# EtherealEngine/Universal-Volumetric

Measured on AMD Instinct MI355X. Metric: frames/s encode, 100k-vert mesh + 2048^2 texture, higher is better.
Workload: dtype u8/int32 (f32 only in the quantiser)

## Files before the change

### universal-volumetric_amd/csrc/tex_encode.hip

```cpp
#include "uvol_common.hpp"
#include "tex_device.hpp"
#include <algorithm>

#define TJOB_OR_RETURN TexJob &J = job[blockIdx.z]; if (J.status != 0) return
#define TEX_RETRY_ALPHA (~(size_t)0)

__device__ inline uint32_t t_block_excl_scan(uint32_t v, uint32_t *total) {
  __shared__ uint32_t wsum[UVOL_BLOCK / 64];
  const int lane = threadIdx.x & 63, w = threadIdx.x >> 6;
  uint32_t x = v;
  for (int d = 1; d < 64; d <<= 1) { uint32_t y = __shfl_up(x, d); if (lane >= d) x += y; }
  if (lane == 63) wsum[w] = x;
  __syncthreads();
  uint32_t base = 0, tot = 0;
  for (int i = 0; i < UVOL_BLOCK / 64; i++) { if (i < w) base += wsum[i]; tot += wsum[i]; }
  __syncthreads();
  *total = tot;
  return base + x - v;
}
__global__ void __launch_bounds__(UVOL_BLOCK) k_tscan_a(TexJob *job, uint32_t n) {
  TexJob &J = job[blockIdx.z];
  const uint32_t i = blockIdx.x * UVOL_BLOCK + threadIdx.x;
  uint32_t v = (J.status == 0 && i < n) ? J.flag[i] : 0, tot;
  t_block_excl_scan(v, &tot);
  if (threadIdx.x == 0) J.bsum[blockIdx.x] = tot;
}
__global__ void __launch_bounds__(UVOL_BLOCK) k_tscan_b(TexJob *job, uint32_t nblocks) {
  TexJob &J = job[blockIdx.z];
  __shared__ uint32_t carry;
  if (threadIdx.x == 0) carry = 0;
  __syncthreads();
  for (uint32_t b0 = 0; b0 < nblocks; b0 += UVOL_BLOCK) {
    const uint32_t i = b0 + threadIdx.x;
    uint32_t v = i < nblocks ? J.bsum[i] : 0, tot;
    const uint32_t ex = t_block_excl_scan(v, &tot);
    const uint32_t c = carry;
    if (i < nblocks) J.bsum[i] = c + ex;
    __syncthreads();
    if (threadIdx.x == 0) carry = c + tot;
    __syncthreads();
  }
  if (threadIdx.x == 0) J.bsum[nblocks] = carry;
}

__global__ void __launch_bounds__(UVOL_BLOCK) k_tex_skip(TexJob *job) {
  TJOB_OR_RETURN;
  const uint32_t b = blockIdx.x * UVOL_BLOCK + threadIdx.x;
  if (b >= J.nb) return;
  const uint32_t X = b % J.bx, Y = b / J.bx;
  uint32_t anchor[16], cur[16], amask = 0xff000000u;
  const uint32_t st = 1u << J.ashift;
  for (uint32_t kind = 0; kind < st; kind++) {
    t_load_block(J, kind, X, Y, anchor, &amask);
    J.skip[(size_t)kind * J.nb + b] = 0; J.flag[(size_t)kind * J.nb + b] = 1;
    for (uint32_t l = kind + st; l < J.L; l += st) {
      t_load_block(J, l, X, Y, cur, &amask);
      uint32_t d = 0;
      for (int i = 0; i < 16; i++) {
        const int dr = (int)(cur[i] & 255) - (int)(anchor[i] & 255), dg = (int)((cur[i] >> 8) & 255) - (int)((anchor[i] >> 8) & 255), db = (int)((cur[i] >> 16) & 255) - (int)((anchor[i] >> 16) & 255);
        d += (uint32_t)(dr * dr + dg * dg + db * db);
      }
      const bool sk = d <= J.T_skip;
      J.skip[(size_t)l * J.nb + b] = sk ? 1 : 0; J.flag[(size_t)l * J.nb + b] = sk ? 0 : 1;
      if (!sk) for (int i = 0; i < 16; i++) anchor[i] = cur[i];
    }
  }
  if (!J.ashift && (amask & 0xff000000u) != 0xff000000u) J.status = TEX_E_ALPHA;
}

__global__ void __launch_bounds__(UVOL_BLOCK) k_tex_fit(TexJob *job) {
  TJOB_OR_RETURN;
  const uint32_t it = blockIdx.x * UVOL_BLOCK + threadIdx.x;
  if (it >= J.n_items) return;
  const uint32_t b = J.item[it];
  const uint32_t l = b / J.nb, r = b % J.nb;
  uint32_t px[16]; t_load_block(J, l, r % J.bx, r / J.bx, px);
  int sum[3] = {0, 0, 0};
  for (int i = 0; i < 16; i++) { sum[0] += (int)(px[i] & 255); sum[1] += (int)((px[i] >> 8) & 255); sum[2] += (int)((px[i] >> 16) & 255); }
  int base5[3]; for (int c = 0; c < 3; c++) base5[c] = (((sum[c] + 8) >> 4) * 31 + 127) / 255;
  uint32_t best = 0xffffffffu; int bc0 = 0, bc1 = 0, bc2 = 0, bt = 0;
  for (int t = 0; t < 8; t++) for (int di = 0; di < 3; di++) {
    const int dd = di == 0 ? 0 : (di == 1 ? -1 : 1);
    const int c0 = t_clampi(base5[0] + dd, 0, 31), c1 = t_clampi(base5[1] + dd, 0, 31), c2 = t_clampi(base5[2] + dd, 0, 31);
    const uint32_t e = t_eval_block<false, false>(px, c0, c1, c2, t, nullptr, nullptr);
    if (e < best) { best = e; bt = t; bc0 = c0; bc1 = c1; bc2 = c2; }
  }
  for (int c = 0; c < 3; c++) for (int di = 1; di < 3; di++) {
    const int dd = di == 1 ? -1 : 1;
    int c0 = bc0 + (c == 0 ? dd : 0), c1 = bc1 + (c == 1 ? dd : 0), c2 = bc2 + (c == 2 ? dd : 0);
    const int cc = c == 0 ? c0 : (c == 1 ? c1 : c2);
    if (cc < 0 || cc > 31) continue;
    const uint32_t e = t_eval_block<false, false>(px, c0, c1, c2, bt, nullptr, nullptr);
    if (e < best) { best = e; bc0 = c0; bc1 = c1; bc2 = c2; }
  }
  const uint32_t cell = ((uint32_t)bt << 15) | ((uint32_t)bc0 << 10) | ((uint32_t)bc1 << 5) | (uint32_t)bc2;
  J.cell[b] = cell;
  atomicAdd(&J.hist[cell], 1u);
}

__global__ void __launch_bounds__(UVOL_BLOCK) k_cell_flags(TexJob *job) {
  TJOB_OR_RETURN;
  const uint32_t c = blockIdx.x * UVOL_BLOCK + threadIdx.x;
  if (c < (1u << 18)) J.flag[c] = J.hist[c] ? 1 : 0;
}
__global__ void __launch_bounds__(UVOL_BLOCK) k_cell_compact(TexJob *job) {
  TexJob &J = job[blockIdx.z];
  const uint32_t c = blockIdx.x * UVOL_BLOCK + threadIdx.x;
  const bool live = J.status == 0 && c < (1u << 18);
  uint32_t v = live ? J.flag[c] : 0, tot;
  const uint32_t pos = t_block_excl_scan(v, &tot) + J.bsum[blockIdx.x];
  if (live && v) { J.cid[pos] = c; J.cw[pos] = J.hist[c]; J.cidx[c] = pos; }
  if (blockIdx.x == 0 && threadIdx.x == 0 && J.status == 0) {
    const uint32_t n = J.bsum[(1u << 18) / UVOL_BLOCK];
    J.ncell = n;
    TexVQ &V = J.vq[0]; V.n_items = n; V.K = n < J.Kmax_e ? n : J.Kmax_e; V.nl = 1; V.done = (V.K <= 1) ? 1 : 0;
  }
}

template <int DIM> __device__ __forceinline__ void vq_item(const TexJob &J, uint32_t i, int x[DIM], unsigned long long &w) {
  if (DIM == 4) { t_cell_coords(J.cid[i], x); w = J.cw[i]; }
  else { const uint32_t s = J.bsel[J.item[i]]; for (int k = 0; k < DIM; k++) x[k] = (int)((s >> (2 * k)) & 3); w = 1; }
}
template <int DIM> __device__ __forceinline__ int vq_wd(int d) { return (DIM == 4 && d == 3) ? 2 : 1; }

template <int DIM>
__global__ void __launch_bounds__(UVOL_BLOCK) k_vq_zero(TexJob *job, int force) {
  TJOB_OR_RETURN;
  TexVQ &V = J.vq[DIM == 4 ? 0 : 1];
  if (V.done && !force) return;
  const uint32_t i = blockIdx.x * UVOL_BLOCK + threadIdx.x;
// ... 236 lines not shown
  }
  if (live) V.leaf[i] = bk;
}

__global__ void __launch_bounds__(UVOL_BLOCK) k_unique(TexJob *job, int which) {
  TJOB_OR_RETURN;
  const uint32_t K = J.vq[which].nl;
  const uint32_t *val = which == 0 ? J.ent : J.scb;
  uint32_t *outv = which == 0 ? J.ecb : J.scu, *map = which == 0 ? J.emap : J.smap;
  uint8_t *first = J.vq[which].splittable;
  __shared__ uint32_t s_cnt;
  if (threadIdx.x == 0) s_cnt = 0;
  __syncthreads();
  for (uint32_t k = threadIdx.x; k < K; k += UVOL_BLOCK) {
    const bool used = which == 0 ? (J.vq[0].stW[k] != 0) : (J.sused[k] != 0);
    uint8_t f = 0;
    if (used) { f = 1; const uint32_t v = val[k]; for (uint32_t j = 0; j < k; j++) { const bool uj = which == 0 ? (J.vq[0].stW[j] != 0) : (J.sused[j] != 0); if (uj && val[j] == v) { f = 2; break; } } }
    first[k] = f;
  }
  __syncthreads();
  uint32_t mine = 0;
  for (uint32_t k = threadIdx.x; k < K; k += UVOL_BLOCK) {
    if (!first[k]) { map[k] = 0; continue; }
    const uint32_t v = val[k]; uint32_t less = 0;
    for (uint32_t j = 0; j < K; j++) less += (first[j] == 1 && val[j] < v) ? 1u : 0u;
    map[k] = less;
    if (first[k] == 1) { outv[less] = v; mine++; }
  }
  if (mine) atomicAdd(&s_cnt, mine);
  __syncthreads();
  if (threadIdx.x == 0) { if (which == 0) J.ne = s_cnt; else J.ns = s_cnt; }
}

__global__ void __launch_bounds__(UVOL_BLOCK) k_block_assign(TexJob *job) {
  TJOB_OR_RETURN;
  const uint32_t it = blockIdx.x * UVOL_BLOCK + threadIdx.x;
  if (it >= J.n_items) return;
  const uint32_t b = J.item[it];
  const uint32_t cl = J.vq[0].leaf[J.cidx[J.cell[b]]], tup = J.ent[cl];
  J.bei[b] = (uint16_t)J.emap[cl];
  const uint32_t l = b / J.nb, r = b % J.nb;
  uint32_t px[16]; t_load_block(J, l, r % J.bx, r / J.bx, px);
  uint32_t sel;
  t_eval_block<true, false>(px, (int)((tup >> 10) & 31), (int)((tup >> 5) & 31), (int)(tup & 31), (int)(tup >> 15), &sel, nullptr);
  J.bsel[b] = sel;
}
__global__ void __launch_bounds__(UVOL_BLOCK) k_item_compact(TexJob *job) {
  TexJob &J = job[blockIdx.z];
  const uint32_t b = blockIdx.x * UVOL_BLOCK + threadIdx.x;
  const bool live = J.status == 0 && b < J.NB;
  uint32_t v = live ? J.flag[b] : 0, tot;
  const uint32_t pos = t_block_excl_scan(v, &tot) + J.bsum[blockIdx.x];
  if (live && v) { J.item[pos] = b; J.vq[1].leaf[pos] = 0; }
  if (blockIdx.x == 0 && threadIdx.x == 0 && J.status == 0) {
    const uint32_t n = J.bsum[(J.NB + UVOL_BLOCK - 1) / UVOL_BLOCK];
    J.n_items = n;
    TexVQ &V = J.vq[1]; V.n_items = n; V.K = n < J.Kmax_s ? n : J.Kmax_s; V.nl = 1; V.done = (V.K <= 1) ? 1 : 0;
  }
}
__global__ void __launch_bounds__(UVOL_BLOCK) k_cell_leaf_init(TexJob *job) {
  TJOB_OR_RETURN;
  const uint32_t i = blockIdx.x * UVOL_BLOCK + threadIdx.x;
  if (i < J.vq[0].n_items) J.vq[0].leaf[i] = 0;
}

__global__ void __launch_bounds__(UVOL_BLOCK) k_sel_centroids(TexJob *job) {
  TJOB_OR_RETURN;
  TexVQ &V = J.vq[1];
  const uint32_t k = blockIdx.x * UVOL_BLOCK + threadIdx.x;
  if (k >= V.nl) return;
  const long long W = (long long)V.stW[k]; if (!W) return;
  uint32_t v = 0;
  for (int d = 0; d < 16; d++) v |= (uint32_t)((2 * (long long)V.stS[(size_t)k * 16 + d] + W) / (2 * W)) << (2 * d);
  J.scb[k] = v;
}
#define SA_CHUNK 512u
__global__ void __launch_bounds__(UVOL_BLOCK) k_sel_assign(TexJob *job) {
  TJOB_OR_RETURN;
  TexVQ &V = J.vq[1];
  if (blockIdx.x * UVOL_BLOCK >= V.n_items) return;
  __shared__ uint32_t lds[SA_CHUNK * 16];
  const uint32_t tid = threadIdx.x, lane = tid & 63u, wv = tid >> 6, i = blockIdx.x * UVOL_BLOCK + tid;
  {
    unsigned long long rows[16];
    for (int t = 0; t < 16; t++) rows[t] = 0;
    if (i < V.n_items) {
      const uint32_t b = J.item[i], tup = J.ecb[J.bei[b]];
      const uint32_t l = b / J.nb, r = b % J.nb;
      uint32_t px[16]; t_load_block(J, l, r % J.bx, r / J.bx, px);
      t_eval_block<false, true>(px, (int)((tup >> 10) & 31), (int)((tup >> 5) & 31), (int)(tup & 31), (int)(tup >> 15), nullptr, rows);
    }
    const uint32_t tile = lane >> 4, x = lane & 15u;
    for (int t = 0; t < 16; t++) {
      const uint32_t lo32 = (uint32_t)rows[t], hi32 = (uint32_t)(rows[t] >> 32);
      const uint32_t lo = (lo32 & 0xffu) | ((lo32 >> 8) & 0xff00u) | ((hi32 & 0xffu) << 16) | ((hi32 << 8) & 0xff000000u);
      const uint32_t hi = ((lo32 >> 8) & 0xffu) | ((lo32 >> 16) & 0xff00u) | ((hi32 << 8) & 0xff0000u) | (hi32 & 0xff000000u);
      const uint32_t g = (uint32_t)t >> 2, w = (uint32_t)t & 3u;
      lds[((((wv * 4 + tile) * 2 + 0) * 4 + g) * 16 + x) * 4 + w] = lo ^ 0x80808080u;
      lds[((((wv * 4 + tile) * 2 + 1) * 4 + g) * 16 + x) * 4 + w] = hi ^ 0x80808080u;
    }
  }
  __syncthreads();
  uint32_t blo[4][4], bhi[4][4], best[4];
  for (uint32_t tile = 0; tile < 4; tile++) {
    const uint32_t o0 = (((wv * 4 + tile) * 2 + 0) * 64 + lane) * 4, o1 = (((wv * 4 + tile) * 2 + 1) * 64 + lane) * 4;
    for (int w = 0; w < 4; w++) { blo[tile][w] = lds[o0 + w]; bhi[tile][w] = lds[o1 + w]; }
    best[tile] = 0xffffffffu;
  }
  const uint32_t nl = V.nl;
  for (uint32_t c0 = 0; c0 < nl; c0 += SA_CHUNK) {
    const uint32_t cn = nl - c0 < SA_CHUNK ? nl - c0 : SA_CHUNK, ctn = (cn + 15u) >> 4;
    __syncthreads();
    for (uint32_t idx = tid; idx < ctn * 256u; idx += UVOL_BLOCK) {
      const uint32_t ct = idx >> 8, rem = idx & 255u, g = rem >> 6, x = (rem >> 2) & 15u, w = rem & 3u;
      uint32_t k = c0 + ct * 16 + x; if (k >= nl) k = nl - 1;
      lds[idx] = 1u << (8u * ((J.scb[k] >> (2u * (4u * g + w))) & 3u));
    }
    __syncthreads();
    uint32_t kbr[4];
    for (uint32_t r = 0; r < 4; r++) { kbr[r] = c0 + 4 * (lane >> 4) + r; UVOL_OPAQUE(kbr[r]); }
    for (uint32_t ct = 0; ct < ctn; ct++) {
      uint32_t a[4];
      for (int w = 0; w < 4; w++) a[w] = lds[(ct * 64 + lane) * 4 + w];
#pragma unroll
      for (int tile = 0; tile < 4; tile++) {
        int H[4] = { 2048, 2048, 2048, 2048 }, L[4] = { 2048, 2048, 2048, 2048 };
        t_mfma_i8_16x16x64(a, bhi[tile], H);
        t_mfma_i8_16x16x64(a, blo[tile], L);
#pragma unroll
        for (int r = 0; r < 4; r++) {
          uint32_t d = ((uint32_t)H[r] << 8) + (uint32_t)L[r];
          UVOL_OPAQUE(d);
          const uint32_t key = (d << 11) | kbr[r];
          best[tile] = key < best[tile] ? key : best[tile];
        }
      }
      for (uint32_t r = 0; r < 4; r++) kbr[r] += 16;
    }
  }
  for (uint32_t tile = 0; tile < 4; tile++) {
    uint32_t m = best[tile], o;
    o = __shfl_xor(m, 16); m = o < m ? o : m;
    o = __shfl_xor(m, 32); m = o < m ? o : m;
    const uint32_t it = blockIdx.x * UVOL_BLOCK + wv * 64 + tile * 16 + (lane & 15u);
    if (lane < 16 && it < V.n_items) V.leaf[it] = m & 2047u;
  }
}
__global__ void __launch_bounds__(UVOL_BLOCK) k_sel_used(TexJob *job, int phase) {
  TJOB_OR_RETURN;
  TexVQ &V = J.vq[1];
  const uint32_t i = blockIdx.x * UVOL_BLOCK + threadIdx.x;
  if (phase == 0) { if (i < V.K) J.sused[i] = 0; }
  else if (phase == 1) { if (i < V.n_items) J.sused[V.leaf[i]] = 1; }
  else { if (i < V.n_items) J.bsi[J.item[i]] = (uint16_t)J.smap[V.leaf[i]]; }
}
__global__ void __launch_bounds__(UVOL_BLOCK) k_copy_skipped(TexJob *job) {
  TJOB_OR_RETURN;
  const uint32_t b = blockIdx.x * UVOL_BLOCK + threadIdx.x;
  if (b >= J.nb) return;
  uint32_t nsk = 0;
  const uint32_t st = 1u << J.ashift;
  for (uint32_t l = st; l < J.L; l++) {
    const size_t o = (size_t)l * J.nb + b, pv = o - (size_t)st * J.nb;
    if (J.skip[o]) { J.bei[o] = J.bei[pv]; J.bsi[o] = J.bsi[pv]; nsk++; }
  }
  if (nsk) atomicAdd(&J.n_skipped, nsk);
}

__device__ __forceinline__ uint32_t t_pred_of(const TexJob &J, uint32_t l, uint32_t x, uint32_t y) {
  const size_t o = (size_t)l * J.nb; const uint32_t b = y * J.bx + x;
  const uint16_t *ei = J.bei + o;
  if (J.skip[o + b]) return 2;
  if (x > 0 && ei[b] == ei[b - 1]) return 0;
  if (y > 0 && ei[b] == ei[b - J.bx]) return 1;
  if ((l >> J.ashift) == 0 && x > 0 && y > 0 && ei[b] == ei[b - J.bx - 1]) return 2;
  return 3;
}
__global__ void __launch_bounds__(UVOL_BLOCK) k_preds(TexJob *job) {
// ... 312 lines not shown
      tb_put(w, 0, 1); tb_put(w, 0, 1); tb_put(w, 0, 1);
      J.hm[8].n = 256; for (int i = 0; i < 256; i++) J.hm[8].freq[i] = 0;
      for (uint32_t k = 1; k < ns; k++) for (int j = 0; j < 4; j++) J.hm[8].freq[((J.scu[k] >> (8 * j)) ^ (J.scu[k - 1] >> (8 * j))) & 255]++;
      uint32_t s = 0; for (int i = 0; i < 256; i++) s |= J.hm[8].freq[i]; if (!s) J.hm[8].freq[0] = 1;
    }
    __syncthreads();
    dev_huff_build(J.hm[8].freq, 256, 16, J.hm[8].size, J.hm[8].code, scratch);
    dev_write_huff(w, J.hm[8].size, 256, scratch);
    if (threadIdx.x == 0) {
      for (int j = 0; j < 4; j++) tb_put(w, (J.scu[0] >> (8 * j)) & 255, 8);
      for (uint32_t k = 1; k < ns; k++) for (int j = 0; j < 4; j++) { const uint32_t s = ((J.scu[k] >> (8 * j)) ^ (J.scu[k - 1] >> (8 * j))) & 255; tb_put(w, J.hm[8].code[s], J.hm[8].size[s]); }
    }
  } else {
    for (int m = 0; m < 4; m++) dev_write_huff(w, J.hm[m].size, (int)J.hm[m].n, scratch);
    if (threadIdx.x == 0) tb_put(w, TEX_HS, 13);
  }
  __syncthreads();
  if (threadIdx.x == 0) { tb_flush(w); J.sec_len[sec] = w.n; if (w.overflow) J.status = -50; }
}

__device__ __forceinline__ void t_tok_bits(const TexJob &J, unsigned long long tk, unsigned long long &bits, uint32_t &len) {
  const uint32_t kind = (uint32_t)(tk & 255), sym = (uint32_t)((tk >> 8) & 0xffffff), extra = (uint32_t)(tk >> 32);
  bits = 0; len = 0;
  if (kind == 255) return;
  const int mi = kind <= 1 ? 0 : (kind == 2 ? 1 : 2);
  const uint32_t s0 = kind == 1 ? 256u : (kind == 4 ? J.ns + TEX_HS : sym);
  bits = J.hm[mi].code[s0]; len = J.hm[mi].size[s0];
  if (kind == 1) { unsigned long long vb; int vl; t_vlc(extra, 4, vb, vl); bits |= vb << len; len += (uint32_t)vl; }
  else if (kind == 4) {
    bits |= (unsigned long long)J.hm[3].code[sym] << len; len += J.hm[3].size[sym];
    if (sym == 63) { unsigned long long vb; int vl; t_vlc(extra, 7, vb, vl); bits |= vb << len; len += (uint32_t)vl; }
  }
}
__global__ void __launch_bounds__(UVOL_BLOCK) k_pack_a(TexJob *job) {
  TexJob &J = job[blockIdx.z];
  const uint32_t l = blockIdx.y, i = blockIdx.x * UVOL_BLOCK + threadIdx.x, n = 3 * J.nb;
  unsigned long long bits; uint32_t len = 0;
  if (J.status == 0 && i < n) t_tok_bits(J, J.tok[3 * (size_t)l * J.nb + i], bits, len);
  uint32_t tot; t_block_excl_scan(len, &tot);
  if (threadIdx.x == 0) J.bsum[(size_t)l * (gridDim.x + 1) + blockIdx.x] = tot;
}
__global__ void __launch_bounds__(UVOL_BLOCK) k_pack_b(TexJob *job, uint32_t nblocks) {
  TexJob &J = job[blockIdx.z];
  const uint32_t l = blockIdx.x;
  uint32_t *bs = J.bsum + (size_t)l * (nblocks + 1);
  __shared__ uint32_t carry;
  if (threadIdx.x == 0) carry = 0;
  __syncthreads();
  for (uint32_t b0 = 0; b0 < nblocks; b0 += UVOL_BLOCK) {
    const uint32_t i = b0 + threadIdx.x;
    uint32_t v = i < nblocks ? bs[i] : 0, tot;
    const uint32_t ex = t_block_excl_scan(v, &tot);
    const uint32_t c = carry;
    if (i < nblocks) bs[i] = c + ex;
    __syncthreads();
    if (threadIdx.x == 0) carry = c + tot;
    __syncthreads();
  }
  if (threadIdx.x == 0) {
    bs[nblocks] = carry;
    if (J.status == 0) { J.slice_bits[l] = carry; J.slice_len[l] = (carry + 7) / 8; if ((carry + 7) / 8 + 8 > J.slice_cap) J.status = -51; }
  }
}
__global__ void __launch_bounds__(UVOL_BLOCK) k_pack_c(TexJob *job) {
  TexJob &J = job[blockIdx.z];
  const uint32_t l = blockIdx.y, i = blockIdx.x * UVOL_BLOCK + threadIdx.x, n = 3 * J.nb;
  unsigned long long bits = 0; uint32_t len = 0;
  const bool ok = J.status == 0;
  if (ok && i < n) t_tok_bits(J, J.tok[3 * (size_t)l * J.nb + i], bits, len);
  uint32_t tot;
  const uint32_t off = t_block_excl_scan(len, &tot) + (ok ? J.bsum[(size_t)l * (gridDim.x + 1) + blockIdx.x] : 0);
  if (!ok || len == 0) return;
  uint32_t *out = reinterpret_cast<uint32_t *>(J.slice[l]);
  const uint32_t wi = off >> 5, sh = off & 31;
  const unsigned long long lo = bits << sh;
  atomicOr(&out[wi], (uint32_t)lo);
  if (sh + len > 32) atomicOr(&out[wi + 1], (uint32_t)(lo >> 32));
  if (sh + len > 64) atomicOr(&out[wi + 2], (uint32_t)(bits >> (64 - sh)));
}

__global__ void k_tex_pack_offsets(TexJob *job, int n_seg) {
  if (threadIdx.x != 0 || blockIdx.x != 0) return;
  unsigned long long off = 0;
  for (int s = 0; s < n_seg; s++) {
    TexJob &J = job[s];
    unsigned long long len = 0;
    if (J.status == 0) { for (int k = 0; k < 3; k++) len += J.sec_len[k]; for (uint32_t l = 0; l < J.L; l++) len += J.slice_len[l]; }
    J.pack_off = off; J.pack_len = len; off += (len + 15ull) & ~15ull;
  }
}
__global__ void __launch_bounds__(UVOL_BLOCK) k_tex_pack(TexJob *job, uint8_t *packed, unsigned long long cap) {
  TJOB_OR_RETURN;
  if (J.pack_off + J.pack_len > cap) return;
  uint8_t *dst = packed + J.pack_off;
  const size_t stride = (size_t)gridDim.x * UVOL_BLOCK, t0 = (size_t)blockIdx.x * UVOL_BLOCK + threadIdx.x;
  for (uint32_t p = 0; p < 3 + J.L; p++) {
    const uint8_t *src = p < 3 ? J.sec[p] : J.slice[p - 3]; const uint32_t len = p < 3 ? J.sec_len[p] : J.slice_len[p - 3];
    for (size_t i = t0; i < len; i += stride) dst[i] = src[i];
    dst += len;
  }
}

struct TexLane {
  hipStream_t stream = nullptr; bool own_stream = false;
  uvol_devbuf slab, layers, job, packed;
  std::vector<TexJob> hjobs;
  uint8_t *pinned = nullptr; size_t pinned_cap = 0;
  int n_seg = 0, n_layers = 0, alpha = 0; uint32_t W = 0, H = 0;
  uint8_t *const *outs = nullptr; const size_t *caps = nullptr; size_t *out_lens = nullptr;
  int *status = nullptr;
  bool busy = false, on_device = false;
  std::vector<uint8_t *> outv; std::vector<size_t> capv; std::vector<const uint8_t *> srcv;
  UvolUpSlot *up = nullptr; uint64_t up_gen = 0; std::vector<size_t> up_off;
};
struct TexState { TexLane lane[2]; int next = 0; int deferred_rc = UVOL_OK; char deferred_err[512] = {0}; };
int tex_create(uvol_ctx *ctx) { ctx->tex = new TexState(); ctx->tex->lane[0].stream = ctx->stream; return UVOL_OK; }
void tex_destroy(uvol_ctx *ctx) {
  if (!ctx->tex) return;
  for (TexLane &t : ctx->tex->lane) {
    if (t.own_stream && t.stream) { (void)hipStreamSynchronize(t.stream); (void)hipStreamDestroy(t.stream); }
    for (uvol_devbuf *b : { &t.slab, &t.packed, &t.layers, &t.job }) if (b->p) (void)hipFree(b->p);
    if (t.pinned) (void)hipHostFree(t.pinned);
  }
  delete ctx->tex; ctx->tex = nullptr;
}
int tex_trim(uvol_ctx *ctx) {
  TexState *T = ctx->tex; if (!T) return UVOL_OK;
  for (TexLane &t : T->lane) {
    if (t.busy) continue;
    if (t.stream) UVOL_HIP_CHECK(ctx, hipStreamSynchronize(t.stream));
    for (uvol_devbuf *b : { &t.slab, &t.packed, &t.layers }) if (b->p) { UVOL_HIP_CHECK(ctx, hipFree(b->p)); b->p = nullptr; b->cap = 0; }
  }
  return UVOL_OK;
}
size_t uvol_texture_bound(uint32_t w, uint32_t h, int n) {
  const size_t nb = (size_t)((w + 3) / 4) * ((h + 3) / 4);
  return 65536 + 6 * (size_t)TEX_MAX_CODEBOOK * 4 + (nb * 16 + 64) * (size_t)(n > 0 ? n : 1);
}

namespace {
struct TCarver { size_t off = 0; template <class T> size_t take(size_t count) { off = (off + 255) & ~(size_t)255; size_t o = off; off += count * sizeof(T); return o; } };
size_t tex_layout(TexJob &J, uint8_t *base, size_t *zero_bytes) {
  TCarver C;
  const size_t NB = J.NB, nb = J.nb, KC = TEX_MAX_CODEBOOK;
#define TCARVE(field, T, count) do { size_t o_ = C.take<T>(count); if (base) field = (T *)(base + o_); } while (0)
  TCARVE(J.hist, uint32_t, (size_t)1 << 18);
  for (int m = 0; m < TEX_NMODEL; m++) TCARVE(J.hm[m].freq, uint32_t, TEX_MODEL_CAP);
  TCARVE(J.ent, uint32_t, KC + 8); TCARVE(J.scb, uint32_t, KC + 8);
  for (uint32_t l = 0; l < J.L; l++) TCARVE(J.slice[l], uint8_t, J.slice_cap);
  *zero_bytes = (C.off + 255) & ~(size_t)255;
  TCARVE(J.skip, uint8_t, NB + 8); TCARVE(J.cell, uint32_t, NB + 8);
  const size_t nflag = std::max<size_t>(NB, (size_t)1 << 18) + 8;
  TCARVE(J.flag, uint8_t, nflag);
  const size_t nbs = std::max<size_t>(nflag / UVOL_BLOCK + 8, (size_t)J.L * ((3 * nb + UVOL_BLOCK - 1) / UVOL_BLOCK + 2));
  TCARVE(J.bsum, uint32_t, nbs);
  TCARVE(J.cid, uint32_t, (size_t)1 << 18); TCARVE(J.cw, uint32_t, (size_t)1 << 18); TCARVE(J.cidx, uint32_t, (size_t)1 << 18);
  for (int v = 0; v < 2; v++) {
    TexVQ &V = J.vq[v]; const size_t dim = v == 0 ? 4 : 16, ni = v == 0 ? ((size_t)1 << 18) : NB;
    TCARVE(V.leaf, uint32_t, ni + 8);
    TCARVE(V.stW, unsigned long long, KC + 8); TCARVE(V.stS, unsigned long long, (KC + 8) * dim); TCARVE(V.stQ, unsigned long long, (KC + 8) * dim);
    TCARVE(V.splittable, uint8_t, KC + 8); TCARVE(V.chosen, uint8_t, KC + 8); TCARVE(V.axis, int32_t, KC + 8);
    TCARVE(V.th, long long, KC + 8); TCARVE(V.prio, long long, KC + 8); TCARVE(V.newidx, uint32_t, KC + 8); TCARVE(V.split, uint32_t, KC + 8);
  }
  TCARVE(J.ecb, uint32_t, KC + 8); TCARVE(J.emap, uint32_t, KC + 8);
  TCARVE(J.bei, uint16_t, NB + 8); TCARVE(J.bsi, uint16_t, NB + 8); TCARVE(J.bsel, uint32_t, NB + 8);
  TCARVE(J.item, uint32_t, NB + 8);
  TCARVE(J.sused, uint8_t, KC + 8); TCARVE(J.scu, uint32_t, KC + 8); TCARVE(J.smap, uint32_t, KC + 8);
  TCARVE(J.pred, uint8_t, NB + 8);
  TCARVE(J.clist, uint32_t, NB + 8); TCARVE(J.msym, uint8_t, NB + 8); TCARVE(J.gid, uint32_t, NB + 8); TCARVE(J.gstart, uint32_t, NB + 8); TCARVE(J.gsize, uint32_t, NB + 8);
  TCARVE(J.tok, unsigned long long, 3 * NB + 8);
  for (int m = 0; m < TEX_NMODEL; m++) { TCARVE(J.hm[m].size, uint8_t, TEX_MODEL_CAP); TCARVE(J.hm[m].code, uint16_t, TEX_MODEL_CAP); }
  TCARVE(J.hscratch, uint32_t, (size_t)7 * 10 * (TEX_MODEL_CAP + 8));
  for (int s = 0; s < 3; s++) { J.sec_cap[s] = (uint32_t)(6 * KC * 4 + 4096); TCARVE(J.sec[s], uint8_t, J.sec_cap[s]); }
#undef TCARVE
  return (C.off + 255) & ~(size_t)255;
}
inline void put32(uint8_t *&p, uint32_t v) { memcpy(p, &v, 4); p += 4; }
inline void put64(uint8_t *&p, uint64_t v) { memcpy(p, &v, 8); p += 8; }
inline void put16(uint8_t *&p, uint16_t v) { memcpy(p, &v, 2); p += 2; }
}

#define TLAUNCH(k, grid, block, shmem, ...)                                                      \
  do {                                                                                           \
    if (uvol_debug()) { fprintf(stderr, "[uvol] launch %s\n", #k); fflush(stderr); }              \
    dim3 g3_ = grid; g3_.z = NSEG;                                                               \
    hipLaunchKernelGGL(k, g3_, block, shmem, ctx->stream, __VA_ARGS__);                          \
    if (uvol_debug()) { hipError_t e_ = hipStreamSynchronize(ctx->stream); if (e_ != hipSuccess) { fprintf(stderr, "[uvol] %s FAILED: %s\n", #k, hipGetErrorString(e_)); fflush(stderr); } } \
  } while (0)

static inline unsigned vq_stat_blocks(unsigned item_blocks, unsigned nseg) {
  const unsigned per = std::max(32u, std::min(512u, 4096u / std::max(1u, nseg)));
  return std::min(item_blocks, per);
}
template <int DIM, int LCAP, typename CT>
static void run_vq_rounds(uvol_ctx *ctx, TexJob *dj, unsigned item_blocks, unsigned NSEG, uint32_t kmax) {
  const unsigned kb = uvol_blocks((size_t)TEX_MAX_CODEBOOK * DIM);
  const unsigned sb = vq_stat_blocks(item_blocks, NSEG);
  TLAUNCH((k_vq_zero<DIM>), dim3(kb), dim3(UVOL_BLOCK), 0, dj, 0);
  for (int r = 0; r < TEX_VQ_ROUNDS; r++) {
    const uint32_t leaves_r = r < 20 ? std::min<uint32_t>(kmax, 1u << r) : kmax, lds_leaves = std::min<uint32_t>((uint32_t)LCAP, std::max<uint32_t>(leaves_r, 16u));
    for (uint32_t lb = 0; lb < leaves_r; lb += LCAP) TLAUNCH((k_vq_stats<DIM, LCAP, CT>), dim3(sb), dim3(UVOL_BLOCK), (size_t)lds_leaves * (1 + 2 * DIM) * sizeof(CT), dj, 0, lb, lds_leaves);
    TLAUNCH((k_vq_decide<DIM, false>), dim3(1), dim3(UVOL_BLOCK), 0, dj, 0);
    TLAUNCH((k_vq_apply<DIM>), dim3(item_blocks), dim3(UVOL_BLOCK), 0, dj);
  }
}
template <int DIM, int LCAP, typename CT>
static void run_vq_stats(uvol_ctx *ctx, TexJob *dj, unsigned item_blocks, unsigned NSEG, uint32_t kmax) {
  const size_t shmem = (size_t)LCAP * (1 + 2 * DIM) * sizeof(CT);
  TLAUNCH((k_vq_zero<DIM>), dim3(uvol_blocks((size_t)TEX_MAX_CODEBOOK * DIM)), dim3(UVOL_BLOCK), 0, dj, 1);
  for (uint32_t lb = 0; lb < kmax; lb += LCAP) TLAUNCH((k_vq_stats<DIM, LCAP, CT>), dim3(vq_stat_blocks(item_blocks, NSEG)), dim3(UVOL_BLOCK), shmem, dj, 1, lb, (uint32_t)LCAP);
}

static inline uint32_t sel_lcap_max() { static const uint32_t v = [] { const char *e = getenv("UVOL_SEL_LCAP"); const int x = e ? atoi(e) : 0; return (uint32_t)(x >= 16 && x <= 768 ? x : 256); }(); return v; }
static inline uint32_t sel_lcap(const TexJob &J) { const uint32_t cap = std::min<uint32_t>(sel_lcap_max(), 448u); return J.Kmax_s < cap ? J.Kmax_s : cap; }
typedef unsigned long long sel_word_t;
static inline unsigned sel_stat_blocks(const TexJob &J, unsigned nseg) { return std::min(std::max(32u, std::min(512u, 4096u / std::max(1u, nseg))), std::max(1u, (unsigned)((J.NB + UVOL_BLOCK * SEL_ILP - 1) / (UVOL_BLOCK * SEL_ILP)))); }
static void run_sel_stats(uvol_ctx *ctx, TexJob *dj, const TexJob &J, unsigned NSEG, int force, int round = -1) {
  const uint32_t leaves = (round >= 0 && round < 20) ? std::min<uint32_t>(J.Kmax_s, std::max<uint32_t>(1u << round, 16u)) : J.Kmax_s;
  const uint32_t lcap = std::min<uint32_t>(sel_lcap(J), leaves);
  if (force) TLAUNCH((k_vq_zero<16>), dim3(uvol_blocks((size_t)TEX_MAX_CODEBOOK * 16)), dim3(UVOL_BLOCK), 0, dj, force);
// ... 26 lines not shown
  J0.yflip = ctx->prm.y_flip ? 1 : 0;
  const int q = std::min(255, std::max(1, ctx->prm.etc1s_quality));
  J0.Kmax_e = (uint32_t)std::min(TEX_MAX_CODEBOOK, std::max(32, q * 12)); J0.Kmax_s = (uint32_t)std::min(TEX_MAX_CODEBOOK, std::max(32, q * 6));
  J0.T_skip = (uint32_t)((255 - q) * 3 / 2);
  J0.slice_cap = (uint32_t)((size_t)J0.nb * 8 + 64);
  size_t zero_bytes = 0; const size_t ws = tex_layout(J0, nullptr, &zero_bytes);
  const size_t lbytes = (size_t)W * H * 4;
  int rc;
  if ((rc = uvol_ensure(ctx, L.slab, ws * (size_t)n_seg))) return rc;
  if ((rc = uvol_ensure(ctx, L.job, sizeof(TexJob) * (size_t)n_seg))) return rc;
  const bool pre_up = !on_device && L.up != nullptr;
  if (!on_device && !pre_up && (rc = uvol_ensure(ctx, L.layers, lbytes * (size_t)n_layers * (size_t)n_seg))) return rc;
  L.hjobs.assign((size_t)n_seg, J0);
  std::vector<UvolUpItem> ups;
  for (int s = 0; s < n_seg; s++) {
    TexJob &J = L.hjobs[s];
    uint8_t *base = (uint8_t *)L.slab.p + ws * (size_t)s;
    tex_layout(J, base, &zero_bytes);
    UVOL_HIP_CHECK(ctx, hipMemsetAsync(base, 0, zero_bytes, ctx->stream));
    for (int l = 0; l < n_layers; l++) {
      const uint8_t *src = rgba[(size_t)s * n_layers + l];
      if (on_device) J.layer[l] = src;
      else if (pre_up) J.layer[l] = (const uint8_t *)L.up->buf.p + L.up_off[(size_t)s * n_layers + l];
      else { uint8_t *d = (uint8_t *)L.layers.p + lbytes * ((size_t)s * n_layers + l); ups.push_back(UvolUpItem{ lbytes * ((size_t)s * n_layers + l), src, lbytes }); J.layer[l] = d; }
    }
  }
  if (!on_device && !pre_up) { const int rcu = uvol_upload_staged(ctx, (uint8_t *)L.layers.p, ups); if (rcu != UVOL_OK) return rcu; }
  if (pre_up) { const int rcu = uvol_uplink_acquire(ctx, L.up, ctx->stream); if (rcu != UVOL_OK) return rcu; }
  UVOL_HIP_CHECK(ctx, hipMemcpyAsync(L.job.p, L.hjobs.data(), sizeof(TexJob) * (size_t)n_seg, hipMemcpyHostToDevice, ctx->stream));
  TexJob *dj = (TexJob *)L.job.p;
  const TexJob &J = J0;
  const unsigned bnb = uvol_blocks(J.nb), bNB = uvol_blocks(J.NB), bcell = (1u << 18) / UVOL_BLOCK, bK = uvol_blocks(TEX_MAX_CODEBOOK);
  const uint64_t src_bytes = (uint64_t)lbytes * n_layers * (uint64_t)n_seg;
  { uvol_ctx::Scope sc(ctx, "tex.k11_skip", src_bytes); TLAUNCH(k_tex_skip, dim3(bnb), dim3(UVOL_BLOCK), 0, dj);
    TLAUNCH(k_tscan_a, dim3(bNB), dim3(UVOL_BLOCK), 0, dj, J.NB);
    TLAUNCH(k_tscan_b, dim3(1), dim3(UVOL_BLOCK), 0, dj, bNB);
    TLAUNCH(k_item_compact, dim3(bNB), dim3(UVOL_BLOCK), 0, dj); }
  { uvol_ctx::Scope sc(ctx, "tex.k9_endpoint_fit", src_bytes); TLAUNCH(k_tex_fit, dim3(bNB), dim3(UVOL_BLOCK), 0, dj); }
  {
    uvol_ctx::Scope sc(ctx, "tex.k10_endpoint_codebook", 0);
    TLAUNCH(k_cell_flags, dim3(bcell), dim3(UVOL_BLOCK), 0, dj);
    TLAUNCH(k_tscan_a, dim3(bcell), dim3(UVOL_BLOCK), 0, dj, 1u << 18);
    TLAUNCH(k_tscan_b, dim3(1), dim3(UVOL_BLOCK), 0, dj, bcell);
    TLAUNCH(k_cell_compact, dim3(bcell), dim3(UVOL_BLOCK), 0, dj);
    TLAUNCH(k_cell_leaf_init, dim3(bcell), dim3(UVOL_BLOCK), 0, dj);
    run_vq_rounds<4, 256, unsigned long long>(ctx, dj, bcell, NSEG, J.Kmax_e);
    for (int it = 0; it <= 2; it++) {
      run_vq_stats<4, 256, unsigned long long>(ctx, dj, bcell, NSEG, J.Kmax_e);
      TLAUNCH(k_ep_entries, dim3(bK), dim3(UVOL_BLOCK), 0, dj);
      if (it < 2) TLAUNCH(k_ep_assign, dim3(bcell), dim3(UVOL_BLOCK), 0, dj);
    }
    TLAUNCH(k_unique, dim3(1), dim3(UVOL_BLOCK), 0, dj, 0);
  }
  {
    uvol_ctx::Scope sc(ctx, "tex.k9b_block_selectors", src_bytes);
    TLAUNCH(k_block_assign, dim3(bNB), dim3(UVOL_BLOCK), 0, dj);
  }
  {
    uvol_ctx::Scope sc(ctx, "tex.k10_selector_codebook", src_bytes * 2);
    run_sel_rounds(ctx, dj, J, bNB, NSEG);
    for (int it = 0; it < 2; it++) {
      if (it) run_sel_stats(ctx, dj, J, NSEG, 1);
      TLAUNCH(k_sel_centroids, dim3(bK), dim3(UVOL_BLOCK), 0, dj);
      { uvol_ctx::Scope sc2(ctx, "tex.k10_sel_assign", 0); TLAUNCH(k_sel_assign, dim3(bNB), dim3(UVOL_BLOCK), 0, dj); }
    }
    TLAUNCH(k_sel_used, dim3(bK), dim3(UVOL_BLOCK), 0, dj, 0);
    TLAUNCH(k_sel_used, dim3(bNB), dim3(UVOL_BLOCK), 0, dj, 1);
    TLAUNCH(k_unique, dim3(1), dim3(UVOL_BLOCK), 0, dj, 1);
    TLAUNCH(k_sel_used, dim3(bNB), dim3(UVOL_BLOCK), 0, dj, 2);
    TLAUNCH(k_copy_skipped, dim3(bnb), dim3(UVOL_BLOCK), 0, dj);
  }
  const unsigned bslots = uvol_blocks((size_t)3 * J.nb);
  {
    uvol_ctx::Scope sc(ctx, "tex.k12_symbolize", (uint64_t)J.NB * 6 * n_seg);
    TLAUNCH(k_preds, dim3(bNB), dim3(UVOL_BLOCK), 0, dj);
    TLAUNCH(k_tok_delta, dim3(bNB), dim3(UVOL_BLOCK), 0, dj);
    TLAUNCH(k_sscan_a, dim3(bnb, J.L), dim3(UVOL_BLOCK), 0, dj, J.nb, J.nb);
    TLAUNCH(k_sscan_b, dim3(J.L), dim3(UVOL_BLOCK), 0, dj, bnb);
    TLAUNCH(k_coded_list, dim3(bnb, J.L), dim3(UVOL_BLOCK), 0, dj);
    const uint32_t nm = ((J.bx + 1) / 2) * ((J.by + 1) / 2); const unsigned bnm = uvol_blocks(nm);
    TLAUNCH(k_mb_flags, dim3(bnm, J.L), dim3(UVOL_BLOCK), 0, dj, nm);
    TLAUNCH(k_sscan_a, dim3(bnm, J.L), dim3(UVOL_BLOCK), 0, dj, nm, nm);
    TLAUNCH(k_sscan_b, dim3(J.L), dim3(UVOL_BLOCK), 0, dj, bnm);
    TLAUNCH(k_mb_groups, dim3(bnm, J.L), dim3(UVOL_BLOCK), 0, dj, nm);
    TLAUNCH(k_mb_tokens, dim3(bnm, J.L), dim3(UVOL_BLOCK), 0, dj, nm);
    { uvol_ctx::Scope sc2(ctx, "tex.k12_sel_tokens", (uint64_t)J.NB * 6 * n_seg); TLAUNCH(k_sel_tokens, dim3(J.L), dim3(64), 0, dj); }
    const size_t lh_bytes = (size_t)(257 + J.Kmax_e + J.Kmax_s + TEX_HS + 1 + 64) * 4;
    if (lh_bytes > 60 * 1024) { ctx->set_error("etc1s_quality too high for the LDS histogram (codebooks > 60 KiB)"); return UVOL_E_UNSUPPORTED; }
    TLAUNCH(k_tok_hist, dim3(std::min<unsigned>(uvol_blocks((size_t)3 * J.NB), 1024u)), dim3(UVOL_BLOCK), lh_bytes, dj);
  }
  {
    uvol_ctx::Scope sc(ctx, "tex.k12_huffman_pack", (uint64_t)J.NB * 24 * n_seg);
    TLAUNCH(k_huff_models, dim3(4), dim3(UVOL_BLOCK), 0, dj);
    TLAUNCH(k_sections, dim3(3), dim3(UVOL_BLOCK), 0, dj);
    TLAUNCH(k_pack_a, dim3(bslots, J.L), dim3(UVOL_BLOCK), 0, dj);
    TLAUNCH(k_pack_b, dim3(J.L), dim3(UVOL_BLOCK), 0, dj, bslots);
    TLAUNCH(k_pack_c, dim3(bslots, J.L), dim3(UVOL_BLOCK), 0, dj);
  }
  size_t pack_cap = 0;
  { const TexJob &Jc = L.hjobs[0]; pack_cap = (((size_t)Jc.sec_cap[0] + Jc.sec_cap[1] + Jc.sec_cap[2] + (size_t)Jc.slice_cap * (size_t)Jc.L) + 15) & ~(size_t)15; }
  size_t want_pack = std::max<size_t>(L.packed.cap, pack_cap * (size_t)n_seg / 8 + 4096);
  if (int rc = uvol_ensure(ctx, L.packed, want_pack)) return rc;
  { uvol_ctx::Scope sc(ctx, "tex.k13_pack", 0);
    hipLaunchKernelGGL(k_tex_pack_offsets, dim3(1), dim3(64), 0, ctx->stream, dj, n_seg);
    TLAUNCH(k_tex_pack, dim3(32), dim3(UVOL_BLOCK), 0, dj, (uint8_t *)L.packed.p, (unsigned long long)L.packed.cap); }
  UVOL_HIP_CHECK(ctx, hipGetLastError());
  if (pre_up) { const int rcr = uvol_uplink_release(ctx, L.up, ctx->stream); if (rcr != UVOL_OK) return rcr; }
  return UVOL_OK;
}
static int tex_finish_impl(uvol_ctx *ctx, TexLane &L) {
  const int n_seg = L.n_seg, n_layers = L.n_layers, alpha = L.alpha; const uint32_t W = L.W, H = L.H;
  uint8_t *const *outs = L.outs; const size_t *caps = L.caps; size_t *out_lens = L.out_lens;
  if (n_seg <= 0) return UVOL_OK;
  TexJob *dj = (TexJob *)L.job.p; const unsigned NSEG = (unsigned)n_seg;
  UVOL_HIP_CHECK(ctx, hipStreamSynchronize(ctx->stream));
  UVOL_HIP_CHECK(ctx, hipMemcpy(L.hjobs.data(), dj, sizeof(TexJob) * (size_t)n_seg, hipMemcpyDeviceToHost));
  if (ctx->profiling) {
    uint64_t ops = 0;
    for (int s = 0; s < n_seg; s++) { const TexVQ &V = L.hjobs[s].vq[1]; ops += 2ull * (uint64_t)V.n_items * (uint64_t)((V.nl + 15u) & ~15u) * 64ull * 2ull * 2ull; }
    ctx->prof[ctx->prof_index("tex.k10_sel_assign")].algo_bytes += ops;
  }
  size_t packed_total = 0;
  for (int s = 0; s < n_seg; s++) packed_total = std::max<size_t>(packed_total, (size_t)(L.hjobs[s].pack_off + ((L.hjobs[s].pack_len + 15ull) & ~15ull)));
  if (packed_total > L.packed.cap) {
    if (int rc = uvol_ensure(ctx, L.packed, packed_total)) return rc;
    TLAUNCH(k_tex_pack, dim3(32), dim3(UVOL_BLOCK), 0, dj, (uint8_t *)L.packed.p, (unsigned long long)L.packed.cap);
    UVOL_HIP_CHECK(ctx, hipGetLastError());
  }
  if (packed_total > L.pinned_cap) {
    if (L.pinned) (void)hipHostFree(L.pinned);
// ... 158 lines not shown
```

Before: 3529.

## Convert texture block kernels to bounded grid-stride walks over segments

Five texture kernels (skip, fit, block assign, selector assign, pack a/c) are rewritten to use a TexWalk helper. The helper either runs one block per grid slot when the launch grid is full, or strides over a flattened (segment, y, x) space when the grid is capped. The fit and selector-assign kernels are capped at CU count times 4, so early-exit blocks for segments with few live items are skipped in bulk instead of each being launched. The light kernels keep the full grid by default, since their weight is 0. The change adds a CU-count query and an environment override, and risks less parallelism when the walk is capped.

```diff
diff --git a/universal-volumetric_amd/csrc/tex_encode.hip b/universal-volumetric_amd/csrc/tex_encode.hip
--- a/universal-volumetric_amd/csrc/tex_encode.hip
+++ b/universal-volumetric_amd/csrc/tex_encode.hip
@@ -4,6 +4,22 @@
 
 #define TJOB_OR_RETURN TexJob &J = job[blockIdx.z]; if (J.status != 0) return
 #define TEX_RETRY_ALPHA (~(size_t)0)
+
+struct TexWalk {
+  uint32_t v, end, stride, bx, bps, seg, y, x; bool full;
+  __device__ TexWalk(uint32_t bx_, uint32_t by, uint32_t nseg) : bx(bx_), bps(bx_ * by) {
+    full = gridDim.x == bx && gridDim.y == by && gridDim.z == nseg;
+    end = bps * nseg; stride = gridDim.x; v = full ? 0u : blockIdx.x;
+  }
+  __device__ bool more() {
+    if (full) { seg = blockIdx.z; y = blockIdx.y; x = blockIdx.x; return v == 0u; }
+    if (v >= end) return false;
+    seg = v / bps; const uint32_t r = v - seg * bps; y = bx == bps ? 0u : r / bx; x = r - y * bx;
+    return true;
+  }
+  __device__ void next() { v = full ? 1u : v + stride; }
+  __device__ void next_segment() { v = full ? 1u : v + ((seg + 1u) * bps - v + stride - 1u) / stride * stride; }
+};
 
 __device__ inline uint32_t t_block_excl_scan(uint32_t v, uint32_t *total) {
   __shared__ uint32_t wsum[UVOL_BLOCK / 64];
@@ -43,10 +59,7 @@
   if (threadIdx.x == 0) J.bsum[nblocks] = carry;
 }
 
-__global__ void __launch_bounds__(UVOL_BLOCK) k_tex_skip(TexJob *job) {
-  TJOB_OR_RETURN;
-  const uint32_t b = blockIdx.x * UVOL_BLOCK + threadIdx.x;
-  if (b >= J.nb) return;
+__device__ __forceinline__ void t_skip_block(TexJob &J, uint32_t b) {
   const uint32_t X = b % J.bx, Y = b / J.bx;
   uint32_t anchor[16], cur[16], amask = 0xff000000u;
   const uint32_t st = 1u << J.ashift;
@@ -67,11 +80,15 @@
   }
   if (!J.ashift && (amask & 0xff000000u) != 0xff000000u) J.status = TEX_E_ALPHA;
 }
-
-__global__ void __launch_bounds__(UVOL_BLOCK) k_tex_fit(TexJob *job) {
-  TJOB_OR_RETURN;
-  const uint32_t it = blockIdx.x * UVOL_BLOCK + threadIdx.x;
-  if (it >= J.n_items) return;
+__global__ void __launch_bounds__(UVOL_BLOCK) k_tex_skip(TexJob *job, uint32_t bps, uint32_t nseg) {
+  for (TexWalk w(bps, 1, nseg); w.more(); w.next()) {
+    TexJob &J = job[w.seg];
+    const uint32_t b = w.x * UVOL_BLOCK + threadIdx.x;
+    if (J.status == 0 && b < J.nb) t_skip_block(J, b);
+  }
+}
+
+__device__ __forceinline__ void t_fit_block(TexJob &J, uint32_t it) {
   const uint32_t b = J.item[it];
   const uint32_t l = b / J.nb, r = b % J.nb;
   uint32_t px[16]; t_load_block(J, l, r % J.bx, r / J.bx, px);
@@ -96,6 +113,15 @@
   const uint32_t cell = ((uint32_t)bt << 15) | ((uint32_t)bc0 << 10) | ((uint32_t)bc1 << 5) | (uint32_t)bc2;
   J.cell[b] = cell;
   atomicAdd(&J.hist[cell], 1u);
+}
+__global__ void __launch_bounds__(UVOL_BLOCK) k_tex_fit(TexJob *job, uint32_t bps, uint32_t nseg) {
+  for (TexWalk w(bps, 1, nseg); w.more();) {
+    TexJob &J = job[w.seg];
+    if (J.status != 0 || w.x * UVOL_BLOCK >= J.n_items) { w.next_segment(); continue; }
+    const uint32_t it = w.x * UVOL_BLOCK + threadIdx.x;
+    if (it < J.n_items) t_fit_block(J, it);
+    w.next();
+  }
 }
 
 __global__ void __launch_bounds__(UVOL_BLOCK) k_cell_flags(TexJob *job) {
@@ -398,10 +424,7 @@
   if (threadIdx.x == 0) { if (which == 0) J.ne = s_cnt; else J.ns = s_cnt; }
 }
 
-__global__ void __launch_bounds__(UVOL_BLOCK) k_block_assign(TexJob *job) {
-  TJOB_OR_RETURN;
-  const uint32_t it = blockIdx.x * UVOL_BLOCK + threadIdx.x;
-  if (it >= J.n_items) return;
+__device__ __forceinline__ void t_assign_block(TexJob &J, uint32_t it) {
   const uint32_t b = J.item[it];
   const uint32_t cl = J.vq[0].leaf[J.cidx[J.cell[b]]], tup = J.ent[cl];
   J.bei[b] = (uint16_t)J.emap[cl];
@@ -410,6 +433,15 @@
   uint32_t sel;
   t_eval_block<true, false>(px, (int)((tup >> 10) & 31), (int)((tup >> 5) & 31), (int)(tup & 31), (int)(tup >> 15), &sel, nullptr);
   J.bsel[b] = sel;
+}
+__global__ void __launch_bounds__(UVOL_BLOCK) k_block_assign(TexJob *job, uint32_t bps, uint32_t nseg) {
+  for (TexWalk w(bps, 1, nseg); w.more();) {
+    TexJob &J = job[w.seg];
+    if (J.status != 0 || w.x * UVOL_BLOCK >= J.n_items) { w.next_segment(); continue; }
+    const uint32_t it = w.x * UVOL_BLOCK + threadIdx.x;
+    if (it < J.n_items) t_assign_block(J, it);
+    w.next();
+  }
 }
 __global__ void __launch_bounds__(UVOL_BLOCK) k_item_compact(TexJob *job) {
   TexJob &J = job[blockIdx.z];
@@ -441,12 +473,9 @@
   J.scb[k] = v;
 }
 #define SA_CHUNK 512u
-__global__ void __launch_bounds__(UVOL_BLOCK) k_sel_assign(TexJob *job) {
-  TJOB_OR_RETURN;
-  TexVQ &V = J.vq[1];
-  if (blockIdx.x * UVOL_BLOCK >= V.n_items) return;
+__device__ __forceinline__ void t_sel_assign_block(TexJob &J, TexVQ &V, uint32_t blk) {
   __shared__ uint32_t lds[SA_CHUNK * 16];
-  const uint32_t tid = threadIdx.x, lane = tid & 63u, wv = tid >> 6, i = blockIdx.x * UVOL_BLOCK + tid;
+  const uint32_t tid = threadIdx.x, lane = tid & 63u, wv = tid >> 6, i = blk * UVOL_BLOCK + tid;
   {
     unsigned long long rows[16];
     for (int t = 0; t < 16; t++) rows[t] = 0;
@@ -508,8 +537,18 @@
     uint32_t m = best[tile], o;
     o = __shfl_xor(m, 16); m = o < m ? o : m;
     o = __shfl_xor(m, 32); m = o < m ? o : m;
-    const uint32_t it = blockIdx.x * UVOL_BLOCK + wv * 64 + tile * 16 + (lane & 15u);
+    const uint32_t it = blk * UVOL_BLOCK + wv * 64 + tile * 16 + (lane & 15u);
     if (lane < 16 && it < V.n_items) V.leaf[it] = m & 2047u;
+  }
+}
+__global__ void __launch_bounds__(UVOL_BLOCK) k_sel_assign(TexJob *job, uint32_t bps, uint32_t nseg) {
+  for (TexWalk w(bps, 1, nseg); w.more();) {
+    TexJob &J = job[w.seg];
+    TexVQ &V = J.vq[1];
+    if (J.status != 0 || w.x * UVOL_BLOCK >= V.n_items) { w.next_segment(); continue; }
+    t_sel_assign_block(J, V, w.x);
+    __syncthreads();
+    w.next();
   }
 }
 __global__ void __launch_bounds__(UVOL_BLOCK) k_sel_used(TexJob *job, int phase) {
@@ -888,13 +927,15 @@
     if (sym == 63) { unsigned long long vb; int vl; t_vlc(extra, 7, vb, vl); bits |= vb << len; len += (uint32_t)vl; }
   }
 }
-__global__ void __launch_bounds__(UVOL_BLOCK) k_pack_a(TexJob *job) {
-  TexJob &J = job[blockIdx.z];
-  const uint32_t l = blockIdx.y, i = blockIdx.x * UVOL_BLOCK + threadIdx.x, n = 3 * J.nb;
-  unsigned long long bits; uint32_t len = 0;
-  if (J.status == 0 && i < n) t_tok_bits(J, J.tok[3 * (size_t)l * J.nb + i], bits, len);
-  uint32_t tot; t_block_excl_scan(len, &tot);
-  if (threadIdx.x == 0) J.bsum[(size_t)l * (gridDim.x + 1) + blockIdx.x] = tot;
+__global__ void __launch_bounds__(UVOL_BLOCK) k_pack_a(TexJob *job, uint32_t bslots, uint32_t L, uint32_t nseg) {
+  for (TexWalk w(bslots, L, nseg); w.more(); w.next()) {
+    TexJob &J = job[w.seg];
+    const uint32_t l = w.y, blk = w.x, i = blk * UVOL_BLOCK + threadIdx.x, n = 3 * J.nb;
+    unsigned long long bits; uint32_t len = 0;
+    if (J.status == 0 && i < n) t_tok_bits(J, J.tok[3 * (size_t)l * J.nb + i], bits, len);
+    uint32_t tot; t_block_excl_scan(len, &tot);
+    if (threadIdx.x == 0) J.bsum[(size_t)l * (bslots + 1) + blk] = tot;
+  }
 }
 __global__ void __launch_bounds__(UVOL_BLOCK) k_pack_b(TexJob *job, uint32_t nblocks) {
   TexJob &J = job[blockIdx.z];
@@ -918,21 +959,23 @@
     if (J.status == 0) { J.slice_bits[l] = carry; J.slice_len[l] = (carry + 7) / 8; if ((carry + 7) / 8 + 8 > J.slice_cap) J.status = -51; }
   }
 }
-__global__ void __launch_bounds__(UVOL_BLOCK) k_pack_c(TexJob *job) {
-  TexJob &J = job[blockIdx.z];
-  const uint32_t l = blockIdx.y, i = blockIdx.x * UVOL_BLOCK + threadIdx.x, n = 3 * J.nb;
-  unsigned long long bits = 0; uint32_t len = 0;
-  const bool ok = J.status == 0;
-  if (ok && i < n) t_tok_bits(J, J.tok[3 * (size_t)l * J.nb + i], bits, len);
-  uint32_t tot;
-  const uint32_t off = t_block_excl_scan(len, &tot) + (ok ? J.bsum[(size_t)l * (gridDim.x + 1) + blockIdx.x] : 0);
-  if (!ok || len == 0) return;
-  uint32_t *out = reinterpret_cast<uint32_t *>(J.slice[l]);
-  const uint32_t wi = off >> 5, sh = off & 31;
-  const unsigned long long lo = bits << sh;
-  atomicOr(&out[wi], (uint32_t)lo);
-  if (sh + len > 32) atomicOr(&out[wi + 1], (uint32_t)(lo >> 32));
-  if (sh + len > 64) atomicOr(&out[wi + 2], (uint32_t)(bits >> (64 - sh)));
+__global__ void __launch_bounds__(UVOL_BLOCK) k_pack_c(TexJob *job, uint32_t bslots, uint32_t L, uint32_t nseg) {
+  for (TexWalk w(bslots, L, nseg); w.more(); w.next()) {
+    TexJob &J = job[w.seg];
+    const uint32_t l = w.y, blk = w.x, i = blk * UVOL_BLOCK + threadIdx.x, n = 3 * J.nb;
+    unsigned long long bits = 0; uint32_t len = 0;
+    const bool ok = J.status == 0;
+    if (ok && i < n) t_tok_bits(J, J.tok[3 * (size_t)l * J.nb + i], bits, len);
+    uint32_t tot;
+    const uint32_t off = t_block_excl_scan(len, &tot) + (ok ? J.bsum[(size_t)l * (bslots + 1) + blk] : 0);
+    if (!ok || len == 0) continue;
+    uint32_t *out = reinterpret_cast<uint32_t *>(J.slice[l]);
+    const uint32_t wi = off >> 5, sh = off & 31;
+    const unsigned long long lo = bits << sh;
+    atomicOr(&out[wi], (uint32_t)lo);
+    if (sh + len > 32) atomicOr(&out[wi + 1], (uint32_t)(lo >> 32));
+    if (sh + len > 64) atomicOr(&out[wi + 2], (uint32_t)(bits >> (64 - sh)));
+  }
 }
 
 __global__ void k_tex_pack_offsets(TexJob *job, int n_seg) {
@@ -969,8 +1012,15 @@
   std::vector<uint8_t *> outv; std::vector<size_t> capv; std::vector<const uint8_t *> srcv;
   UvolUpSlot *up = nullptr; uint64_t up_gen = 0; std::vector<size_t> up_off;
 };
-struct TexState { TexLane lane[2]; int next = 0; int deferred_rc = UVOL_OK; char deferred_err[512] = {0}; };
-int tex_create(uvol_ctx *ctx) { ctx->tex = new TexState(); ctx->tex->lane[0].stream = ctx->stream; return UVOL_OK; }
+struct TexState { TexLane lane[2]; int next = 0; int deferred_rc = UVOL_OK; char deferred_err[512] = {0}; int num_cu = 256; };
+int tex_create(uvol_ctx *ctx) {
+  ctx->tex = new TexState(); ctx->tex->lane[0].stream = ctx->stream;
+#ifndef HIPEMU
+  int v = 0;
+  if (hipDeviceGetAttribute(&v, hipDeviceAttributeMultiprocessorCount, ctx->device) == hipSuccess && v > 0) ctx->tex->num_cu = v;
+#endif
+  return UVOL_OK;
+}
 void tex_destroy(uvol_ctx *ctx) {
   if (!ctx->tex) return;
   for (TexLane &t : ctx->tex->lane) {
@@ -1036,12 +1086,38 @@
 inline void put16(uint8_t *&p, uint16_t v) { memcpy(p, &v, 2); p += 2; }
 }
 
-#define TLAUNCH(k, grid, block, shmem, ...)                                                      \
+#define TLAUNCH_GRID(k, g3, block, shmem, ...)                                                   \
   do {                                                                                           \
     if (uvol_debug()) { fprintf(stderr, "[uvol] launch %s\n", #k); fflush(stderr); }              \
-    dim3 g3_ = grid; g3_.z = NSEG;                                                               \
-    hipLaunchKernelGGL(k, g3_, block, shmem, ctx->stream, __VA_ARGS__);                          \
+    hipLaunchKernelGGL(k, g3, block, shmem, ctx->stream, __VA_ARGS__);                           \
     if (uvol_debug()) { hipError_t e_ = hipStreamSynchronize(ctx->stream); if (e_ != hipSuccess) { fprintf(stderr, "[uvol] %s FAILED: %s\n", #k, hipGetErrorString(e_)); fflush(stderr); } } \
+  } while (0)
+#define TLAUNCH(k, grid, block, shmem, ...) do { dim3 g3_ = grid; g3_.z = NSEG; TLAUNCH_GRID(k, g3_, block, shmem, __VA_ARGS__); } while (0)
+
+#define TEX_W_FIT 4
+#define TEX_W_SEL 4
+#define TEX_W_LIGHT 0
+#define TEX_W_SEL_MAX 4
+#define TEX_EMU_GRID 3u
+enum TexGridClass { TEX_GRID_FIT, TEX_GRID_SEL, TEX_GRID_LIGHT };
+static inline int tex_wgs_env() { static const int v = [] { const char *e = getenv("UVOL_TEX_WGS_PER_CU"); const int x = e && *e ? atoi(e) : -1; return x < 0 ? -1 : std::min(x, 64); }(); return v; }
+static unsigned tex_grid_bound(uvol_ctx *ctx, TexGridClass cls) {
+  const int env = tex_wgs_env();
+#ifdef HIPEMU
+  return env == 0 ? 0u : TEX_EMU_GRID;
+#else
+  const int w = env < 0 ? (cls == TEX_GRID_SEL ? TEX_W_SEL : (cls == TEX_GRID_FIT ? TEX_W_FIT : TEX_W_LIGHT)) : (cls == TEX_GRID_SEL ? std::min(env, TEX_W_SEL_MAX) : env);
+  if (w == 0) return 0;
+  return (unsigned)ctx->tex->num_cu * (unsigned)w;
+#endif
+}
+#define TLAUNCH_WALK(k, cls, dims, ...)                                                           \
+  do {                                                                                           \
+    dim3 g3_ = dims; g3_.z = NSEG;                                                               \
+    if ((unsigned long long)g3_.x * g3_.y * g3_.z >= (1ull << 31)) { ctx->set_error("texture batch: too many blocks for one launch"); return UVOL_E_UNSUPPORTED; } \
+    const unsigned bound_ = tex_grid_bound(ctx, cls);                                            \
+    if (bound_ && (unsigned long long)g3_.x * g3_.y * g3_.z > bound_) g3_ = dim3(bound_);         \
+    TLAUNCH_GRID(k, g3_, dim3(UVOL_BLOCK), 0, __VA_ARGS__);                                      \
   } while (0)
 
 static inline unsigned vq_stat_blocks(unsigned item_blocks, unsigned nseg) {
@@ -1134,11 +1210,11 @@
   const TexJob &J = J0;
   const unsigned bnb = uvol_blocks(J.nb), bNB = uvol_blocks(J.NB), bcell = (1u << 18) / UVOL_BLOCK, bK = uvol_blocks(TEX_MAX_CODEBOOK);
   const uint64_t src_bytes = (uint64_t)lbytes * n_layers * (uint64_t)n_seg;
-  { uvol_ctx::Scope sc(ctx, "tex.k11_skip", src_bytes); TLAUNCH(k_tex_skip, dim3(bnb), dim3(UVOL_BLOCK), 0, dj);
+  { uvol_ctx::Scope sc(ctx, "tex.k11_skip", src_bytes); TLAUNCH_WALK(k_tex_skip, TEX_GRID_LIGHT, dim3(bnb), dj, bnb, NSEG);
     TLAUNCH(k_tscan_a, dim3(bNB), dim3(UVOL_BLOCK), 0, dj, J.NB);
     TLAUNCH(k_tscan_b, dim3(1), dim3(UVOL_BLOCK), 0, dj, bNB);
     TLAUNCH(k_item_compact, dim3(bNB), dim3(UVOL_BLOCK), 0, dj); }
-  { uvol_ctx::Scope sc(ctx, "tex.k9_endpoint_fit", src_bytes); TLAUNCH(k_tex_fit, dim3(bNB), dim3(UVOL_BLOCK), 0, dj); }
+  { uvol_ctx::Scope sc(ctx, "tex.k9_endpoint_fit", src_bytes); TLAUNCH_WALK(k_tex_fit, TEX_GRID_FIT, dim3(bNB), dj, bNB, NSEG); }
   {
     uvol_ctx::Scope sc(ctx, "tex.k10_endpoint_codebook", 0);
     TLAUNCH(k_cell_flags, dim3(bcell), dim3(UVOL_BLOCK), 0, dj);
@@ -1156,7 +1232,7 @@
   }
   {
     uvol_ctx::Scope sc(ctx, "tex.k9b_block_selectors", src_bytes);
-    TLAUNCH(k_block_assign, dim3(bNB), dim3(UVOL_BLOCK), 0, dj);
+    TLAUNCH_WALK(k_block_assign, TEX_GRID_LIGHT, dim3(bNB), dj, bNB, NSEG);
   }
   {
     uvol_ctx::Scope sc(ctx, "tex.k10_selector_codebook", src_bytes * 2);
@@ -1164,7 +1240,7 @@
     for (int it = 0; it < 2; it++) {
       if (it) run_sel_stats(ctx, dj, J, NSEG, 1);
       TLAUNCH(k_sel_centroids, dim3(bK), dim3(UVOL_BLOCK), 0, dj);
-      { uvol_ctx::Scope sc2(ctx, "tex.k10_sel_assign", 0); TLAUNCH(k_sel_assign, dim3(bNB), dim3(UVOL_BLOCK), 0, dj); }
+      { uvol_ctx::Scope sc2(ctx, "tex.k10_sel_assign", 0); TLAUNCH_WALK(k_sel_assign, TEX_GRID_SEL, dim3(bNB), dj, bNB, NSEG); }
     }
     TLAUNCH(k_sel_used, dim3(bK), dim3(UVOL_BLOCK), 0, dj, 0);
     TLAUNCH(k_sel_used, dim3(bNB), dim3(UVOL_BLOCK), 0, dj, 1);
@@ -1195,9 +1271,9 @@
     uvol_ctx::Scope sc(ctx, "tex.k12_huffman_pack", (uint64_t)J.NB * 24 * n_seg);
     TLAUNCH(k_huff_models, dim3(4), dim3(UVOL_BLOCK), 0, dj);
     TLAUNCH(k_sections, dim3(3), dim3(UVOL_BLOCK), 0, dj);
-    TLAUNCH(k_pack_a, dim3(bslots, J.L), dim3(UVOL_BLOCK), 0, dj);
+    TLAUNCH_WALK(k_pack_a, TEX_GRID_LIGHT, dim3(bslots, J.L), dj, bslots, J.L, NSEG);
     TLAUNCH(k_pack_b, dim3(J.L), dim3(UVOL_BLOCK), 0, dj, bslots);
-    TLAUNCH(k_pack_c, dim3(bslots, J.L), dim3(UVOL_BLOCK), 0, dj);
+    TLAUNCH_WALK(k_pack_c, TEX_GRID_LIGHT, dim3(bslots, J.L), dj, bslots, J.L, NSEG);
   }
   size_t pack_cap = 0;
   { const TexJob &Jc = L.hjobs[0]; pack_cap = (((size_t)Jc.sec_cap[0] + Jc.sec_cap[1] + Jc.sec_cap[2] + (size_t)Jc.slice_cap * (size_t)Jc.L) + 15) & ~(size_t)15; }
```

After: 3563, median of 6. About the same (+0.9%).
